# robotseu/ORB_Line_SLAM

Hardware: AMD Instinct MI355X
Metric: stereo frames/s extract+match (ORB+LBD), KITTI 1242x375 (higher is better)
Workload: dtype u8

## Files before the change

### include/orbline.h

```cpp
#ifndef ORBLINE_H
#define ORBLINE_H

#include "orbline_types.h"

#ifdef __cplusplus
extern "C" {
#endif

typedef struct olf_ctx olf_ctx;

const char* olf_last_error(void);
int olf_device_count(void);
int olf_default_params(olf_params* p);

int  olf_ctx_create(const olf_params* p, int width, int height, int max_images, olf_ctx** out);
void olf_ctx_destroy(olf_ctx* ctx);
int  olf_ctx_synchronize(olf_ctx* ctx);
int  olf_ctx_set_input_event(olf_ctx* ctx, void* hip_event);
int  olf_ctx_set_deferred_join(olf_ctx* ctx, int on);
int  olf_stereo_frames_join_dev(olf_ctx* ctx, void* stream);
int  olf_ctx_poll_status(olf_ctx* ctx);

int olf_profile_enable(olf_ctx* ctx, int on);
int olf_profile_reset(olf_ctx* ctx);
// ... 9 lines not shown
                                       float* d_map1, float* d_map2, void* stream);
int olf_init_undistort_rectify_map(olf_ctx* ctx, const double* K, const double* D, int n_dist, const double* R, const double* P, int w, int h,
                                   float* map1, float* map2);
int olf_cvt_gray(olf_ctx* ctx, const uint8_t* src, int code, int n_images, uint8_t* gray);
int olf_remap_linear(olf_ctx* ctx, const uint8_t* src, int src_w, int src_h, const float* mapx, const float* mapy, int dst_w, int dst_h,
                     int n_images, uint8_t* dst);

int olf_distinctive_descriptors(olf_ctx* ctx, const uint8_t* desc, const int32_t* offs, int n_points, int32_t* best);

size_t olf_kf_record_bytes(int n_keys, int n_lines);
int olf_kf_record_pack(uint64_t frame_id, uint64_t kf_id, double timestamp, const float* t3, const float* quat4, int n_keys,
                       const olf_keypoint* keys, const float* uright, const float* depth, const uint8_t* desc, const uint64_t* mappoint_ids,
                       int n_lines, const olf_keyline* lines, const float* disparity2, const double* le3, const uint8_t* ldesc,
                       const uint64_t* mapline_ids, uint8_t* out, size_t capacity, size_t* written);
int olf_kf_record_counts(const uint8_t* buf, size_t len, int32_t* n_keys, int32_t* n_lines, size_t* record_bytes);
int olf_kf_record_unpack(const uint8_t* buf, size_t len, uint64_t* frame_id, uint64_t* kf_id, double* timestamp, float* t3, float* quat4,
                         olf_keypoint* keys, float* uright, float* depth, uint8_t* desc, uint64_t* mappoint_ids, olf_keyline* lines,
                         float* disparity2, double* le3, uint8_t* ldesc, uint64_t* mapline_ids);

typedef struct olf_voc olf_voc;
int olf_voc_create(int k, int L, int scoring, int weighting, int n_nodes, const int32_t* parent, const uint8_t* is_leaf, const uint8_t* desc,
                   const double* weight, olf_voc** out);
int olf_voc_load_text(const char* path, olf_voc** out);
void olf_voc_destroy(olf_voc* voc);
int olf_voc_info(const olf_voc* voc, int* k, int* L, int* scoring, int* weighting, int* n_nodes, int* n_words);
int olf_bow_words_dev(olf_ctx* ctx, const olf_voc* voc, const uint8_t* d_desc, int n, int levelsup, int32_t* d_word, double* d_weight,
                      int32_t* d_node, void* stream);
int olf_bow_assemble(const olf_voc* voc, const int32_t* word, const double* weight, const int32_t* node, int n, int32_t* bow_ids,
                     double* bow_vals, int* n_bow, int32_t* fv_nodes, int32_t* fv_offs, int32_t* fv_idx, int* n_fv);
int olf_bow_transform(olf_ctx* ctx, const olf_voc* voc, const uint8_t* desc, int n, int levelsup, int32_t* bow_ids, double* bow_vals,
                      int* n_bow, int32_t* fv_nodes, int32_t* fv_offs, int32_t* fv_idx, int* n_fv);
int olf_search_by_bow_batch_dev(olf_ctx* ctx, const olf_voc* voc, int n_frames, int img_stride, const olf_keypoint* d_kps, const uint8_t* d_desc,
                                const int32_t* d_counts, const uint8_t* d_mp_valid, const uint8_t* d_mp_bad, float nnratio, int check_orientation,
                                int levelsup, int32_t* d_matches, int32_t* d_nmatches, void* stream);

int olf_orb_scale_tables(const olf_ctx* ctx, float* scale, float* inv_scale, float* sigma2, float* inv_sigma2,
                         int32_t* features_per_level);
int olf_orb_level_sizes(const olf_ctx* ctx, int32_t* widths, int32_t* heights);
int olf_orb_capacity(const olf_ctx* ctx);
int olf_orb_extract_strided(olf_ctx* ctx, const uint8_t* image, size_t row_stride, olf_keypoint* kps, uint8_t* desc, int32_t* count);
int olf_orb_extract_dev(olf_ctx* ctx, const uint8_t* d_images, int n_images, olf_keypoint* d_kps, uint8_t* d_desc,
                        int32_t* d_counts, void* stream);
int olf_orb_extract(olf_ctx* ctx, const uint8_t* images, int n_images, olf_keypoint* kps, uint8_t* desc, int32_t* counts);
int olf_orb_pyramid_level(olf_ctx* ctx, int image, int level, int blurred, uint8_t* dst);
int olf_orb_debug_candidates(olf_ctx* ctx, int image, int level, int32_t* xys, int cap, int32_t* count);
int olf_debug_status(olf_ctx* ctx, int32_t* out64);
int olf_debug_status_n(olf_ctx* ctx, int32_t* out, int n);
int olf_debug_lsd_owner(olf_ctx* ctx, int image, uint32_t* out);
int olf_debug_lsd_regions(olf_ctx* ctx, int image, int32_t* start_n, double* angle, int cap, int32_t* count);
int olf_debug_lsd_waves(olf_ctx* ctx, int waves_per_image, int rob_entries);
int olf_debug_lsd_groups(olf_ctx* ctx, int groups);
int olf_debug_lsd_scatter(olf_ctx* ctx, int on);
int olf_debug_lsd_log_cap(olf_ctx* ctx, int entries);
int olf_debug_seed_sort(olf_ctx* ctx, const uint32_t* keys, int n, int kthr, int depth_limit, uint32_t* out, int32_t* out_n);
int olf_debug_seed_sort_mode(olf_ctx* ctx, int mode);
int olf_debug_seed_sort_wide(olf_ctx* ctx, const uint64_t* keys, int n, int64_t kthr, int depth_limit, int full, uint32_t* out, int32_t* out_n);
int olf_debug_lsd_pool(olf_ctx* ctx, int pool_chunks);
int olf_debug_fdiv_sweep(olf_ctx* ctx, uint64_t seed, int blocks, int per_thread, uint64_t* mismatches);
int olf_debug_sqrtq_sweep(olf_ctx* ctx, int count, uint64_t* mismatches);
int olf_debug_align_sweep(olf_ctx* ctx, uint64_t seed, int blocks, int per_thread, uint64_t* out3);

int olf_stereo_points_dev(olf_ctx* ctx, int n_pairs, const olf_keypoint* d_kps, const uint8_t* d_desc, const int32_t* d_counts,
                          float* d_uright, float* d_depth, void* stream);
int olf_stereo_points(olf_ctx* ctx, const uint8_t* images, int n_pairs, olf_keypoint* kps, uint8_t* desc, int32_t* counts,
                      float* uright, float* depth);

int olf_match_bf_dev(olf_ctx* ctx, const uint8_t* d_descA, const int32_t* d_nA, int strideA, int a_step, const uint8_t* d_descB,
                     const int32_t* d_nB, int strideB, int b_step, int n_sets, float nnr, int best_lr, int32_t* d_m12, void* stream);
int olf_match_bf(olf_ctx* ctx, const uint8_t* descA, int nA, const uint8_t* descB, int nB, float nnr, int best_lr, int32_t* m12);
int olf_knn2(olf_ctx* ctx, const uint8_t* descQ, int nQ, const uint8_t* descT, int nT, int32_t* idx0, int32_t* dist0, int32_t* dist1);
int olf_match_candidates_dev(olf_ctx* ctx, const uint8_t* d_descQ, int nQ, const uint8_t* d_descT, int nT, const int32_t* d_cand_offsets,
                             const int32_t* d_cand_idx, uint16_t* d_dist, void* stream);
int olf_match_candidates(olf_ctx* ctx, const uint8_t* descQ, int nQ, const uint8_t* descT, int nT, const int32_t* cand_offsets,
                         const int32_t* cand_idx, uint16_t* dist);
typedef struct olf_frame_view {
    const olf_keypoint* keys;
    const uint8_t* desc;
    const float*   uright;
    int32_t        n;
    uint8_t*       mp_valid;
    uint8_t*       mp_obs;
    const uint8_t* mp_bad;
    const float*   mp_world;
    const uint8_t* mp_desc;
    const uint8_t* outlier;
    const float*   Tcw;
    float fx, fy, cx, cy, mbf, minX, maxX, minY, maxY;
    const float*   scale_factors;
    int32_t        n_levels;
    const float*   mp_maxd;
    const float*   mp_mind;
    const int32_t* fv_nodes;
    const int32_t* fv_offsets;
    const int32_t* fv_features;
    int32_t        fv_n;
} olf_frame_view;
int olf_search_by_projection(olf_ctx* ctx, const olf_frame_view* cur, const olf_frame_view* last, float th, int bMono, int check_orientation,
                             int32_t* matches, int32_t* nmatches);
int olf_search_by_projection_match12(olf_ctx* ctx, const olf_frame_view* cur, const olf_frame_view* last, float th, int bMono, int check_orientation,
                                     int32_t* matches, int32_t* match12, int32_t* nmatches);
int olf_search_for_initialization(olf_ctx* ctx, const olf_frame_view* f1, const olf_frame_view* f2, float* prev_matched, int window_size,
                                  float nnratio, int check_orientation, int32_t* matches12, int32_t* nmatches);
int olf_search_by_bow(olf_ctx* ctx, const olf_frame_view* kf, const olf_frame_view* f, float nnratio, int check_orientation, int32_t* matched,
                      int32_t* nmatches);
int olf_search_local_map(olf_ctx* ctx, const olf_frame_view* f, int n_mp, const uint8_t* track_in_view, const uint8_t* bad,
                         const int32_t* track_scale_level, const float* track_view_cos, const float* track_proj3, const uint8_t* mp_desc,
// ... 66 lines not shown
```

### orb_line_slam_amd/csrc/api.cpp

```cpp
#include "olf_internal.hpp"
#include "line_internal.hpp"
#include "../../include/orbline.h"
#include <map>
#include <mutex>
#include <cstring>
#include <mutex>

namespace olf {
static thread_local std::string g_err;
void set_error(const std::string& s) { g_err = s; }
}

using namespace olf;

struct olf_ctx {
    olf_params params;
    int W = 0, H = 0, max_images = 0;
    int device = 0;
    hipStream_t stream = nullptr;
    OrbHostTables orb;
    OrbDeviceBufs ob;
    uint8_t* d_images = nullptr;
    olf_keypoint* d_kps = nullptr;
    uint8_t* d_desc = nullptr;
// ... 527 lines not shown
    if (hipMalloc(&b, bytes) != hipSuccess) { (void)hipFree(a); set_error("olf_debug_copy_bandwidth: hipMalloc failed"); return OLF_ERR_HIP; }
    hipEvent_t e0, e1;
    (void)hipEventCreate(&e0); (void)hipEventCreate(&e1);
    (void)hipMemsetAsync(a, 1, bytes, c->stream);
    int rc = olf::launch_copy16(a, b, bytes, c->stream);
    (void)hipEventRecord(e0, c->stream);
    for (int i = 0; i < reps && rc == OLF_OK; ++i) rc = olf::launch_copy16(i & 1 ? b : a, i & 1 ? a : b, bytes, c->stream);
    (void)hipEventRecord(e1, c->stream);
    const hipError_t se = hipEventSynchronize(e1);
    float ms = 0.f;
    (void)hipEventElapsedTime(&ms, e0, e1);
    (void)hipEventDestroy(e0); (void)hipEventDestroy(e1); (void)hipFree(a); (void)hipFree(b);
    if (rc != OLF_OK || se != hipSuccess || !(ms > 0)) { set_error("olf_debug_copy_bandwidth: copy failed"); return OLF_ERR_HIP; }
    *gbytes_per_s = 2.0 * (double)(bytes / 16 * 16) * reps / (ms * 1e-3) / 1e9;
    return OLF_OK;
}

int olf_debug_lsd_waves(olf_ctx* c, int waves_per_image, int rob_entries)
{
    const bool pow2 = rob_entries > 0 && (rob_entries & (rob_entries - 1)) == 0;
    if (!c || waves_per_image > 16 || waves_per_image < -1 || (rob_entries != 0 && (!pow2 || rob_entries < 128 || rob_entries > 1024))) {
        set_error("olf_debug_lsd_waves: bad argument"); return OLF_ERR_INVALID;
    }
    c->lsd_force.waves = waves_per_image;
    c->lsd_force.robEntries = rob_entries;
    return OLF_OK;
}

int olf_debug_lsd_groups(olf_ctx* c, int groups)
{
    if (!c || !(groups == 0 || groups == 1 || groups == 2 || groups == 4)) { set_error("olf_debug_lsd_groups: bad argument"); return OLF_ERR_INVALID; }
    c->lsd_force.groups = groups > 0 ? groups : -1;
    return OLF_OK;
}

int olf_debug_lsd_log_cap(olf_ctx* c, int entries)
{
    if (!c || entries < 0) { set_error("olf_debug_lsd_log_cap: bad argument"); return OLF_ERR_INVALID; }
    OLF_TRY(check_device(c, "olf_debug_lsd_log_cap"));
    LineGeom& g = c->line.geom;
    if (entries > 0 && !g.spillArena) {
        const size_t blocks = std::max<size_t>(2, (size_t)c->max_images - (size_t)c->max_images / 4);
        void* q = nullptr;
        OLF_HIP_CHECK(hipMalloc(&q, blocks * 8 * (size_t)g.Ps));
        c->allocs.push_back(q);
        g.spillArena = static_cast<uint32_t*>(q); g.spillBlocks = (int)blocks;
    }
    g.logCap = entries > 0 ? std::min(entries, g.regionStride / 2) : g.regionStride / 2;
    OLF_HIP_CHECK(hipDeviceSynchronize());
    OLF_HIP_CHECK(hipMemcpy(c->lb.geom, &g, sizeof(LineGeom), hipMemcpyHostToDevice));
    return OLF_OK;
}

int olf_debug_lsd_scatter(olf_ctx* c, int on)
{
    if (!c) { set_error("olf_debug_lsd_scatter: bad argument"); return OLF_ERR_INVALID; }
    c->lsd_force.scatter = on ? 1 : 0;
    return OLF_OK;
}

int olf_debug_seed_sort(olf_ctx* c, const uint32_t* keys, int n, int kthr, int depth_limit, uint32_t* out, int32_t* out_n)
{
    if (!c || !keys || !out || !out_n || n < 0 || n > c->line.geom.Ps || kthr < 0 || kthr > 1023) { set_error("olf_debug_seed_sort: bad argument"); return OLF_ERR_INVALID; }
    OLF_HIP_CHECK(hipMemcpyAsync(c->lb.keysA, keys, (size_t)n * 4, hipMemcpyHostToDevice, c->stream));
    OLF_TRY(launch_lsd_seedsort(c->line.geom, c->lb, lsd_plan(c->line.geom, c->lb, c->lsd_force, c->limits, 1), 1, c->stream, n, kthr, depth_limit));
    int cnt = 0;
    OLF_HIP_CHECK(hipMemcpyAsync(&cnt, c->lb.keyCount, sizeof(int), hipMemcpyDeviceToHost, c->stream));
    OLF_HIP_CHECK(hipStreamSynchronize(c->stream));
    *out_n = cnt;
    if (cnt < 0 || cnt > n) { set_error("olf_debug_seed_sort: count out of range"); return OLF_ERR_HIP; }
    if (cnt) OLF_HIP_CHECK(hipMemcpy(out, c->lb.keysB, (size_t)cnt * 4, hipMemcpyDeviceToHost));
    return OLF_OK;
}

int olf_debug_seed_sort_wide(olf_ctx* c, const uint64_t* keys, int n, int64_t kthr, int depth_limit, int full, uint32_t* out, int32_t* out_n)
{
    if (!c || !keys || !out || !out_n || n < 0 || n > c->line.geom.Ps || kthr < 0 || kthr > 0xffffffffll || !c->line.geom.wide) {
        set_error("olf_debug_seed_sort_wide: bad argument (the context must be a wide one: lsd_n_bins > 1024 or 2^22 pixels and more)"); return OLF_ERR_INVALID; }
    OLF_HIP_CHECK(hipMemcpyAsync(c->lb.keysA, keys, (size_t)n * 8, hipMemcpyHostToDevice, c->stream));
    OLF_TRY(launch_lsd_sort_wide(c->line.geom, c->lb, 1, c->stream, n, (long long)kthr, depth_limit, full ? 1 : 0));
    int cnt = 0;
    OLF_HIP_CHECK(hipMemcpyAsync(&cnt, c->lb.keyCount, sizeof(int), hipMemcpyDeviceToHost, c->stream));
    OLF_HIP_CHECK(hipStreamSynchronize(c->stream));
    *out_n = cnt;
    if (cnt < 0 || cnt > n) { set_error("olf_debug_seed_sort_wide: count out of range"); return OLF_ERR_HIP; }
    if (cnt) OLF_HIP_CHECK(hipMemcpy(out, c->lb.keysB, (size_t)cnt * 4, hipMemcpyDeviceToHost));
    return check_status(c);
}

int olf_debug_seed_sort_mode(olf_ctx* c, int mode)
{
    if (!c || mode < -1 || mode == 3 || mode == 4 || mode > 5) { set_error("olf_debug_seed_sort_mode: bad argument"); return OLF_ERR_INVALID; }
    c->lsd_force.sortMode = mode;
    return OLF_OK;
}

int olf_debug_lsd_pool(olf_ctx* c, int pool_chunks)
{
    if (!c || pool_chunks < 0) { set_error("olf_debug_lsd_pool: bad argument"); return OLF_ERR_INVALID; }
    c->lsd_force.poolChunks = pool_chunks;
    return OLF_OK;
}

int olf_debug_lsd_regions(olf_ctx* c, int image, int32_t* start_n , double* angle, int cap, int32_t* count)
{
    if (!c || !start_n || !angle || !count || image < 0 || image >= c->max_images) return OLF_ERR_INVALID;
// ... 544 lines not shown
```

### orb_line_slam_amd/csrc/line_internal.hpp

```cpp
#pragma once
#include "olf_internal.hpp"

namespace olf {

struct LineGeom {
    int W, H, pitchW;
    int Ws, Hs, pitchS, Ps;
    int nThr;
    int nBins;
    int wide;
    int minRegSize;
    double prec;
    double precWrap;
    double scale;
    double minLength;
    int maxDetect;
    int rectGrid;
    int maxRegions;
    int nFeatures;
    int outCap;
    int pitchD;
    int lsdTaps[7];
    int lsdWideR;
    int lsdWide[15];
// ... 11 lines not shown
    float alignTanLo, alignTanHi;
    float alignDeg;
    int regionStride;
    int resizeExact;
    int logCap;
    int spillBlocks;
    uint32_t* spillArena;
    int* spillCtl;
    int* spillOf;
};

struct LineDeviceBufs {
    uint8_t* lsdBlur = nullptr;
    uint8_t* scaled = nullptr;
    uint32_t* grad = nullptr;
    uint32_t* keysA = nullptr;
    uint32_t* keysB = nullptr;
    int* keyCount = nullptr;
    int* maxN = nullptr;
    int* chunkCnt = nullptr;
    uint32_t* region = nullptr;
    olf_keyline* rawLines = nullptr;
    int* rawCount = nullptr;
    int* regCount = nullptr;
    uint8_t* lbdBlur = nullptr;
    uint32_t* dxdy = nullptr;
    float* rowSums = nullptr;
    float* lbdStarts = nullptr;
    ResizeCoef* rx = nullptr;
    ResizeCoef* ry = nullptr;
    LineGeom* geom = nullptr;
    uint32_t* sortHist = nullptr;
    uint32_t* sortBase = nullptr;
    int* status = nullptr;
    float* angDeg = nullptr;
    void* angEnt = nullptr;
    int ownerImages = 0;
    uint32_t* owner = nullptr;
    int* links = nullptr;
    int nChunks = 0;
    int* growFmt = nullptr;
    int* topBuf = nullptr;
    unsigned char* mg = nullptr;
    size_t mgStride = 0;
    int mgImages = 0;
};

struct LsdOverrides {
    int sortMode = -1;
    int waves = -1, robEntries = 0;
    int groups = -1;
    int poolChunks = 0;
    int scatter = 0;
};

struct DeviceLimits { int nCU = 64, maxLds = 64 * 1024; };

struct LsdPlan {
    enum Resize { Upgrad, Tiled, Upsample } resize;
    enum Sort { Radix, Seed, Wide } sort;
    bool keysOwner, keysAll;
    int sortWaves;
    bool sortTop; int sortGroups;
    int growWaves;
    int robEntries, growGroups, poolChunks, scatter;
    int agentRefine, agentPF, agentLaunches;
    enum Rect { Emit, Mixed, Plain } rect;
};
LsdPlan lsd_plan(const LineGeom& g, const LineDeviceBufs& b, const LsdOverrides& o, const DeviceLimits& d, int n_images);

constexpr int kBatchCtxImages = 2048;

struct LineHostTables {
    LineGeom geom;
    std::vector<ResizeCoef> rx, ry;
    int build(const olf_line_params& p, int W, int H, int max_images = 2);
};

int launch_lsd_front(const LineGeom& g, const LineDeviceBufs& b, const LsdPlan& p, const uint8_t* d_in, int in_pitch, int n_images, hipStream_t s,
                     hipEvent_t sortEvent, bool writeScaled);
int launch_lsd_grow(const LineGeom& g, const LineDeviceBufs& b, const LsdPlan& p, int n_images, hipStream_t s);
int launch_lsd_rect(const LineGeom& g, const LineDeviceBufs& b, const LsdPlan& p, int n_images, hipStream_t s);
int launch_lbd_dense(const LineGeom& g, const LineDeviceBufs& b, const uint8_t* d_in, int in_pitch, int n_images, hipStream_t s);
int launch_line_select_lbd(const LineGeom& g, const LineDeviceBufs& b, const uint8_t* d_in, int in_pitch, int n_images,
                           olf_keyline* d_kls, uint8_t* d_desc, int* d_counts, hipStream_t s, bool denseDone = false);
int launch_lbd_only(const LineGeom& g, const LineDeviceBufs& b, const uint8_t* d_in, int in_pitch, int n_images, const olf_keyline* d_kls,
                    uint8_t* d_desc, const int* d_counts, hipStream_t s);
int launch_gauss7_img(const uint8_t* src, int srcPitch, size_t srcStride, uint8_t* dst, int dstPitch, size_t dstStride, int W, int H,
                      const LineGeom& g, int which, int n_images, hipStream_t s);
int launch_lsd_angle_table(LineDeviceBufs& b, int libmFloat, hipStream_t s);
int launch_fdiv_sweep(unsigned long long seed, int blocks, int per_thread, unsigned long long* d_mismatches, hipStream_t s);
int launch_sqrtq_sweep(int count, unsigned long long* d_mismatches, hipStream_t s);
int launch_align_sweep(const LineDeviceBufs& b, unsigned long long seed, int blocks, int per_thread, unsigned long long* d_out, hipStream_t s);
int lsd_sort_max_chunks(int Ps);
size_t lsd_grow_mg_stride(int maxRegions);
constexpr int kMwMaxImages = 3072;
constexpr int kMgMaxImages = 64;
int launch_lsd_grow_mw(const LineGeom& g, const LineDeviceBufs& b, const LsdPlan& p, int n_images, hipStream_t s);
int lsd_seedsort_top_words();
int launch_lsd_sort(const LineGeom& g, const LineDeviceBufs& b, int n_images, hipStream_t s);
int launch_lsd_seedsort(const LineGeom& g, const LineDeviceBufs& b, const LsdPlan& p, int n_images, hipStream_t s, int nOverride, int kthrOverride, int depthOverride);
int launch_lsd_sort_wide(const LineGeom& g, const LineDeviceBufs& b, int n_images, hipStream_t s, int nOverride, long long kthrOverride, int depthOverride, int fullOverride);

size_t stereo_lines_prep_bytes(int n_images, int cap);
int launch_stereo_lines(int W, int H, const olf_stereo_params& P, int n_pairs, const olf_keyline* d_kls, const uint8_t* d_desc,
                        const int* d_counts, int cap, void* d_prep, uint16_t* d_dist , int* d_m21, int* d_m12,
                        float* d_disp, double* d_le, hipStream_t s);

}
```

### orb_line_slam_amd/csrc/lsd.hip

```cpp
#include "lsd_device.hpp"

namespace olf {


__device__ __forceinline__ int refl101(int p, int n)
{
    if (p < 0) p = -p;
    if (p >= n) p = 2 * (n - 1) - p;
    return p;
}

int launch_gauss7_img(const uint8_t* src, int srcPitch, size_t srcStride, uint8_t* dst, int dstPitch, size_t dstStride, int W, int H,
                      const LineGeom& g, int which, int n_images, hipStream_t s)
{
    if (!which && g.lsdWideR > 3) return launch_sep_wide(src, srcStride, srcPitch, dst, dstStride, dstPitch, W, H, g.lsdWide, g.lsdWideR, n_images, s);
    return launch_sep7(src, srcStride, srcPitch, dst, dstStride, dstPitch, W, H, which ? g.lbdTaps : g.lsdTaps, n_images, s);
}

__global__ __launch_bounds__(256) void k_lsd_upsample(const uint8_t* __restrict__ src, uint8_t* __restrict__ dst,
                                                      const LineGeom* __restrict__ gp, const ResizeCoef* __restrict__ rx,
                                                      const ResizeCoef* __restrict__ ry)
{
    const LineGeom& g = *gp;
    const int img = blockIdx.y;
// ... 1274 lines not shown
                        }
                        ++nreg;
                    } else if (lane == 0) atomicOr(status, 8);
                }
            }
            if (!REFINE && n >= minRegSize) {
                if (nreg < maxRegions) {
                    if (lane == 0) {
                        RegionRec rr; rr.start = rbase; rr.n = n; rr.angle = reg_angle;
                        recs[nreg] = rr;
                    }
                    ++nreg;
                    rbase += n;
                } else if (lane == 0) atomicOr(status, 8);
            }
#ifdef OLF_STATS
            st_acc += n; if (n >= minRegSize) st_logged += n; if (n > 1) st_regl += __popcll(wave_vote(valid && lane > l));
#endif
            if (REFINE && maskEpoch != flushEpoch) {
                const uint32_t wnow = valid ? grad[addr] : kUsed;
                mask = wave_vote(valid && lane > l && !(wnow & (kUsed | kNotDef)) && s_pend[addr & (PEND - 1)] != addr);
                if (wave_bit(mask)) wseed = wnow;
                if (wave_bit(mask & ~tabM) && !isoSeed) { const AngEnt* t = ent + (wseed & 0x3fffffu); seedAng = t->ang; seedSum = t->seed; }
                tabM |= mask;
                maskEpoch = flushEpoch;
            }
            else if (n == 1) mask &= mask - 1;
            else if (PIPE || maskEpoch == flushEpoch) {
                mask &= ~((2ull << l) - 1ull) & wave_vote(s_pend[addr & (PEND - 1)] != addr);
            } else {
                mask = wave_vote(valid && lane > l && !(grad[addr] & (kUsed | kNotDef)) && s_pend[addr & (PEND - 1)] != addr);
                maskEpoch = flushEpoch;
            }
        }
        if (PFSEED) asm volatile("" :: "v"(pfA), "v"(pfB));
    }
#undef ALIGN_CHEAP
#undef ENSURE_ANGLE
#undef LOG_ROOM
#undef LOG_AT
#undef MARK_USED
#undef PEND_FLUSH
#undef PEND_CLEAR
#ifdef OLF_STATS
    if (lane == 0 && img == 0) { long long* o = reinterpret_cast<long long*>(status + 16); o[0] = st_rounds; o[1] = st_k; o[2] = st_t; o[3] = st_full; o[4] = st_single; o[5] = st_rounds_big; o[6] = st_k_big; o[7] = st_t_big;
        o[8] = st_flush; o[9] = st_iters; o[10] = st_deep1; o[11] = st_deep2; o[12] = st_cand; o[13] = st_regions; o[14] = st_mem;
        o[15] = nkeys; o[16] = st_win; o[17] = st_seedl; o[18] = st_regl; o[19] = st_acc; o[20] = st_isos; o[21] = st_logged; o[22] = st_winLive; o[23] = st_first; o[24] = st_cand1;
        o[25] = st_acc1; o[26] = st_wentries; o[27] = st_whand; o[28] = st_wdone; o[29] = st_wpend; }
#endif
    if (lane == 0) { regCount[img] = over ? 0 : nreg; if (growFmt) growFmt[img] = 1; if (g.spillOf && !retry) g.spillOf[img] = over ? -1 : 0; }
}


template <bool CHAINED>
__device__ __forceinline__ void lsd_rect_region(const LineGeom& g, int img, int r, const uint32_t* __restrict__ gradAll,
                                                const uint32_t* __restrict__ regionAll, const RegionRec* __restrict__ recsAll,
                                                SegCand* __restrict__ candAll, const int* __restrict__ linksAll, int nChunks, const int* __restrict__ spillOf,
                                                const uint32_t* __restrict__ spillArena)
{
    const uint32_t* grad = gradAll + (size_t)img * g.Ps;
    const RegionRec rr = recsAll[(size_t)img * g.maxRegions + r];
    const uint32_t* px_list = CHAINED ? regionAll + (size_t)img * nChunks * 32 : nullptr;
    const int sblk = CHAINED || !spillOf ? 0 : spillOf[img];
    const uint2* log2 = CHAINED ? nullptr
                      : (sblk > 0 ? reinterpret_cast<const uint2*>(spillArena) + (size_t)(sblk - 1) * g.Ps
                                  : reinterpret_cast<const uint2*>(regionAll + (size_t)img * g.regionStride)) + rr.start;
    const int* links = CHAINED ? linksAll + (size_t)img * nChunks : nullptr;
    const int n = rr.n, Ws = g.Ws;
    int cid = rr.start, nxt = -1;
#define RECT_BLOCK(q0) (px_list + (size_t)cid * 32 + ((q0) & 31))
#define RECT_STEP(q0) do { if (CHAINED) { if (((q0) & 31) == 0) { if (q0) cid = nxt; nxt = links[cid]; } } } while (0)
    constexpr int U = 16;
    double x = 0, y = 0, sum = 0;
    for (int q0 = 0; q0 < n; q0 += U) {
        uint32_t rp[U], p[U];
        if (CHAINED) {
            RECT_STEP(q0);
            const uint32_t* blk = RECT_BLOCK(q0);
#pragma unroll
            for (int u = 0; u < U; ++u) rp[u] = q0 + u < n ? blk[u] : 0u;
#pragma unroll
            for (int u = 0; u < U; ++u) p[u] = grad[(int)(rp[u] >> 16) * Ws + (int)(rp[u] & 0xffffu)];
        } else {
#pragma unroll
            for (int u = 0; u < U; u += 2) {
                uint4 e = make_uint4(0u, 0u, 0u, 0u);
                if (q0 + u + 1 < n) __builtin_memcpy(&e, log2 + q0 + u, 16);
                else if (q0 + u < n) { const uint2 e1 = log2[q0 + u]; e.x = e1.x; e.y = e1.y; }
                rp[u] = e.x; p[u] = e.y; rp[u + 1] = e.z; p[u + 1] = e.w;
            }
        }
#pragma unroll
        for (int u = 0; u < U; ++u) {
            if (q0 + u < n) {
                const int px = (int)(rp[u] & 0xffffu), py = (int)(rp[u] >> 16);
                const int gx = unpack_gx(p[u]), gy = unpack_gy(p[u]);
                const double wt = sqrt_quarter(gx * gx + gy * gy);
                x = d_add(x, d_mul((double)px, wt));
                y = d_add(y, d_mul((double)py, wt));
                sum = d_add(sum, wt);
            }
        }
    }
    x = x / sum; y = y / sum;
    double Ixx = 0, Iyy = 0, Ixy = 0;
    cid = rr.start;
    for (int q0 = 0; q0 < n; q0 += U) {
        uint32_t rp[U], p[U];
        if (CHAINED) {
            RECT_STEP(q0);
            const uint32_t* blk = RECT_BLOCK(q0);
#pragma unroll
            for (int u = 0; u < U; ++u) rp[u] = q0 + u < n ? blk[u] : 0u;
#pragma unroll
            for (int u = 0; u < U; ++u) p[u] = grad[(int)(rp[u] >> 16) * Ws + (int)(rp[u] & 0xffffu)];
        } else {
#pragma unroll
            for (int u = 0; u < U; u += 2) {
                uint4 e = make_uint4(0u, 0u, 0u, 0u);
                if (q0 + u + 1 < n) __builtin_memcpy(&e, log2 + q0 + u, 16);
                else if (q0 + u < n) { const uint2 e1 = log2[q0 + u]; e.x = e1.x; e.y = e1.y; }
                rp[u] = e.x; p[u] = e.y; rp[u + 1] = e.z; p[u + 1] = e.w;
            }
        }
#pragma unroll
        for (int u = 0; u < U; ++u) {
            if (q0 + u < n) {
                const int px = (int)(rp[u] & 0xffffu), py = (int)(rp[u] >> 16);
                const int gx = unpack_gx(p[u]), gy = unpack_gy(p[u]);
                const double wt = sqrt_quarter(gx * gx + gy * gy);
                const double ex = d_sub((double)px, x), ey = d_sub((double)py, y);
                Ixx = d_add(Ixx, d_mul(d_mul(ey, ey), wt));
                Iyy = d_add(Iyy, d_mul(d_mul(ex, ex), wt));
                Ixy = d_sub(Ixy, d_mul(d_mul(ex, ey), wt));
            }
        }
    }
    const double dI = d_sub(Ixx, Iyy);
    const double lambda = d_mul(0.5, d_sub(d_add(Ixx, Iyy), sqrt(d_add(d_mul(dI, dI), d_mul(d_mul(4.0, Ixy), Ixy)))));
    double theta = (fabs(Ixx) > fabs(Iyy)) ? (double)dev_fastAtan2((float)d_sub(lambda, Ixx), (float)Ixy)
                                           : (double)dev_fastAtan2((float)Ixy, (float)d_sub(lambda, Iyy));
    theta = d_mul(theta, kDegToRads);
    {
        double diff = d_sub(theta, rr.angle);
        while (diff <= -kPI) diff = d_add(diff, kM2PI);
        while (diff > kPI) diff = d_sub(diff, kM2PI);
        if (fabs(diff) > g.prec) theta = d_add(theta, kPI);
    }
    double ddx, ddy;
    sincos(theta, &ddy, &ddx);
    double l_min = 0, l_max = 0;
    cid = rr.start;
    for (int q0 = 0; q0 < n; q0 += U) {
        uint32_t rp[U];
        if (CHAINED) {
            RECT_STEP(q0);
            const uint32_t* blk = RECT_BLOCK(q0);
#pragma unroll
            for (int u = 0; u < U; ++u) rp[u] = q0 + u < n ? blk[u] : 0u;
        } else {
#pragma unroll
            for (int u = 0; u < U; u += 2) {
                uint4 e = make_uint4(0u, 0u, 0u, 0u);
                if (q0 + u + 1 < n) __builtin_memcpy(&e, log2 + q0 + u, 16);
                else if (q0 + u < n) e.x = log2[q0 + u].x;
                rp[u] = e.x; rp[u + 1] = e.z;
            }
        }
#pragma unroll
        for (int u = 0; u < U; ++u) {
            if (q0 + u < n) {
                const double rdx = d_sub((double)(int)(rp[u] & 0xffffu), x), rdy = d_sub((double)(int)(rp[u] >> 16), y);
                const double lq = d_add(d_mul(rdx, ddx), d_mul(rdy, ddy));
                l_max = fmax(l_max, lq); l_min = fmin(l_min, lq);
            }
        }
    }
    double x1 = d_add(x, d_mul(l_min, ddx)), y1 = d_add(y, d_mul(l_min, ddy));
    double x2 = d_add(x, d_mul(l_max, ddx)), y2 = d_add(y, d_mul(l_max, ddy));
    const SegCand c = rect_to_cand(g, x1, y1, x2, y2);
    candAll[(size_t)img * g.maxRegions + r] = c;
#undef RECT_BLOCK
#undef RECT_STEP
}

template <bool CHAINED>
__global__ __launch_bounds__(256) void k_lsd_rect(const LineGeom* __restrict__ gp, const uint32_t* __restrict__ gradAll,
                                                  const uint32_t* __restrict__ regionAll, const RegionRec* __restrict__ recsAll,
                                                  const int* __restrict__ regCount, SegCand* __restrict__ candAll,
                                                  const int* __restrict__ linksAll, int nChunks, const int* __restrict__ spillOf, const uint32_t* __restrict__ spillArena)
{
    const int img = blockIdx.y, r = blockIdx.x * 256 + threadIdx.x;
    if (r >= regCount[img]) return;
    lsd_rect_region<CHAINED>(*gp, img, r, gradAll, regionAll, recsAll, candAll, linksAll, nChunks, spillOf, spillArena);
}

__global__ __launch_bounds__(256) void k_lsd_rect_mixed(const LineGeom* __restrict__ gp, const uint32_t* __restrict__ gradAll,
                                                        const uint32_t* __restrict__ regionAll, const RegionRec* __restrict__ recsAll,
                                                        const int* __restrict__ regCount, SegCand* __restrict__ candAll,
                                                        const int* __restrict__ linksAll, int nChunks, const int* __restrict__ growFmt, const int* __restrict__ spillOf,
                                                        const uint32_t* __restrict__ spillArena)
{
    const int img = blockIdx.y, r = blockIdx.x * 256 + threadIdx.x;
    if (r >= regCount[img]) return;
    if (growFmt[img] == 1) lsd_rect_region<false>(*gp, img, r, gradAll, regionAll, recsAll, candAll, linksAll, nChunks, spillOf, spillArena);
    else lsd_rect_region<true>(*gp, img, r, gradAll, regionAll, recsAll, candAll, linksAll, nChunks, spillOf, spillArena);
}

__global__ __launch_bounds__(256) void k_lsd_emit(const LineGeom* __restrict__ gp, const SegCand* __restrict__ candAll, const int* __restrict__ regCount,
                                                  olf_keyline* __restrict__ rawLines, int* __restrict__ rawCount, int* __restrict__ status)
{
    __shared__ int s_wave[4];
    __shared__ int s_base;
    const LineGeom& g = *gp;
    const int img = blockIdx.x, tid = threadIdx.x, lane = tid & 63, wave = tid >> 6;
    const SegCand* cand = candAll + (size_t)img * g.maxRegions;
    olf_keyline* out = rawLines + (size_t)img * g.maxDetect;
    const int nreg = regCount[img];
    if (tid == 0) s_base = 0;
    __syncthreads();
    for (int r0 = 0; r0 < nreg; r0 += 256) {
        const int r = r0 + tid;
        SegCand c; c.keep = 0;
        if (r < nreg) c = cand[r];
        const unsigned long long km = wave_vote(c.keep != 0);
        if (lane == 0) s_wave[wave] = __popcll(km);
        __syncthreads();
        int pos = s_base + wave_rank_below(km);
        for (int w = 0; w < wave; ++w) pos += s_wave[w];
        if (c.keep) {
            if (pos < g.maxDetect) {
                const float e0 = c.e0, e1 = c.e1, e2 = c.e2, e3 = c.e3;
                olf_keyline kl;
                kl.startPointX = e0; kl.startPointY = e1; kl.endPointX = e2; kl.endPointY = e3;
                kl.sPointInOctaveX = e0; kl.sPointInOctaveY = e1; kl.ePointInOctaveX = e2; kl.ePointInOctaveY = e3;
                kl.lineLength = c.length;
                const int rx1 = __float2int_rn(e0), ry1 = __float2int_rn(e1), rx2 = __float2int_rn(e2), ry2 = __float2int_rn(e3);
                kl.numOfPixels = max(abs(rx2 - rx1), abs(ry2 - ry1)) + 1;
                kl.angle = g.libmFloat ? glibc_atan2f(f_sub(e3, e1), f_sub(e2, e0)) : (float)atan2((double)f_sub(e3, e1), (double)f_sub(e2, e0));
                kl.class_id = pos; kl.octave = 0;
                kl.size = f_mul(f_sub(e2, e0), f_sub(e3, e1));
                kl.response = f_div(kl.lineLength, (float)max(g.W, g.H));
                kl.pt_x = f_div(f_add(e2, e0), 2.0f); kl.pt_y = f_div(f_add(e3, e1), 2.0f);
                out[pos] = kl;
            } else atomicOr(status, 8);
        }
        __syncthreads();
        if (tid == 0) s_base += s_wave[0] + s_wave[1] + s_wave[2] + s_wave[3];
        __syncthreads();
    }
    if (tid == 0) rawCount[img] = min(s_base, g.maxDetect);
}

LsdPlan lsd_plan(const LineGeom& g, const LineDeviceBufs& b, const LsdOverrides& o, const DeviceLimits& d, int n)
{
    LsdPlan p{};
    p.resize = (g.resizeTiled & 4) && g.seedOrder == 1 ? LsdPlan::Upgrad : g.resizeTiled ? LsdPlan::Tiled : LsdPlan::Upsample;
    p.sort = g.wide ? LsdPlan::Wide : g.seedOrder == 1 ? LsdPlan::Seed : LsdPlan::Radix;
    p.keysAll = g.seedOrder == 1;

    const int m = o.sortMode;
    p.sortWaves = m < 0 ? (n <= 256 ? 8 : n <= 640 ? 4 : n <= 1536 ? 2 : 1) : m == 2 ? 8 : m == 1 ? 4 : m == 5 ? 2 : 1;
    auto sortLds = [](int w) { return w == 8 ? 104 * 1024 : w == 4 ? 56 * 1024 : w == 2 ? 32 * 1024 : 0; };
    while (sortLds(p.sortWaves) > d.maxLds) p.sortWaves /= 2;
    p.sortTop = p.sortWaves > 1 && b.topBuf && n <= 64;
    p.sortGroups = !p.sortTop ? 1 : n <= 16 ? 8 : 4;

    const int autoWaves = n <= 512 ? 16 : n <= 1024 ? 8
                        : n <= 1536 ? 4
                        : n <= 2048 ? 8 : n <= kMwMaxImages ? 4
                        : 0;
    p.growWaves = (g.refine || g.wide || n > b.ownerImages) ? 0 : o.waves >= 0 ? o.waves : autoWaves;
    p.keysOwner = p.growWaves > 0;
    if (p.growWaves > 0) {
        const int nw = p.growWaves;
        p.robEntries = o.robEntries > 0 ? o.robEntries : (nw >= 16 ? 512 : nw >= 8 ? 256 : 128);
        p.poolChunks = o.poolChunks > 0 ? std::min(o.poolChunks, b.nChunks) : b.nChunks;
        int G = o.groups > 0 ? o.groups : nw >= 16 && n <= kMgMaxImages ? 2 : 1;
        while (G > 1 && (!b.mg || n > b.mgImages || n * G > d.nCU || p.poolChunks / G < p.robEntries + 64)) G >>= 1;
        p.growGroups = G;
        p.scatter = o.scatter;
        p.agentRefine = 0; p.agentPF = 0; p.agentLaunches = 1;
    } else {
        p.agentRefine = g.refine;
        p.agentPF = (g.wide ? 32 : 0) | (g.refine ? 0 : g.alignTanLo < 0.f ? 11 : 27);
        p.agentLaunches = g.logCap < g.Ps ? 2 : 1;
    }
    p.rect = g.refine ? LsdPlan::Emit : p.growWaves > 0 ? LsdPlan::Mixed : LsdPlan::Plain;
    return p;
}

int launch_lsd_front(const LineGeom& g, const LineDeviceBufs& b, const LsdPlan& p, const uint8_t* d_in, int in_pitch, int n_images, hipStream_t s,
                     hipEvent_t sortEvent, bool writeScaled)
{
    OLF_HIP_CHECK(hipMemsetAsync(b.maxN, 0, (size_t)n_images * 32 * sizeof(int), s));
    OLF_HIP_CHECK(hipMemsetAsync(b.keyCount, 0, (size_t)n_images * 32 * sizeof(int), s));
    { int rc = launch_gauss7_img(d_in, in_pitch, (size_t)in_pitch * g.H, b.lsdBlur, g.pitchW, (size_t)g.pitchW * g.H, g.W, g.H, g, 0, n_images, s);
      if (rc != OLF_OK) return rc; }
    if (p.resize == LsdPlan::Upgrad) {
        const int nsx = (g.Ws + 3) / 4;
        hipLaunchKernelGGL(k_lsd_upgrad, dim3((nsx + 63) / 64, (g.Hs + UG_ROWS - 1) / UG_ROWS, n_images), dim3(64), 0, s, b.lsdBlur, b.scaled, b.grad, b.geom, b.rx, b.ry,
                           b.maxN, nsx, writeScaled ? 1 : 0);
    } else if (p.resize == LsdPlan::Tiled) {
        int rc = launch_resize_tiled(b.lsdBlur, (size_t)g.pitchW * g.H, g.pitchW, g.W, g.H, b.scaled, (size_t)g.pitchS * g.Hs, g.pitchS, g.Ws, g.Hs, b.rx,
                                     b.ry, n_images, s, (g.resizeTiled & 2) != 0);
        if (rc != OLF_OK) return rc;
    } else {
        const int quads = ((g.Ws + 3) >> 2) * g.Hs;
        hipLaunchKernelGGL(k_lsd_upsample, dim3((quads + 255) / 256, n_images), dim3(256), 0, s, b.lsdBlur, b.scaled, b.geom, b.rx, b.ry);
    }
    if (p.resize != LsdPlan::Upgrad) hipLaunchKernelGGL(k_lsd_grad, dim3((g.Ps + LG_CHUNK - 1) / LG_CHUNK, n_images), dim3(256), 0, s, b.scaled, b.grad, b.geom, b.maxN, b.chunkCnt);
    {
        const int nChunks = (g.Ps + LG_CHUNK - 1) / LG_CHUNK, total = nChunks * n_images;
        const size_t lds = (size_t)(LG_CHUNK + 2 * g.Ws + 2) * sizeof(float);
        if (lds > 60 * 1024) { set_error("LSD image wider than the key kernel's LDS window"); return OLF_ERR_CAPACITY; }
        const auto keys = p.sort == LsdPlan::Wide ? (p.keysAll ? k_lsd_keys<false, true, LG_CHUNK, true> : k_lsd_keys<false, false, LG_CHUNK, true>)
                        : p.keysAll ? (p.keysOwner ? k_lsd_keys<true, true, LG_CHUNK> : k_lsd_keys<false, true, LG_CHUNK>)
                        : p.keysOwner ? k_lsd_keys<true, false, LG_CHUNK> : k_lsd_keys<false, false, LG_CHUNK>;
        hipLaunchKernelGGL(keys, dim3(total), dim3(KEYS_THREADS), lds, s, b.grad, b.geom, b.maxN, b.chunkCnt, p.sort == LsdPlan::Radix ? b.keysB : b.keysA, b.keyCount,
                           b.owner, b.angDeg, nChunks, total);
    }
    OLF_HIP_CHECK(hipGetLastError());
    if (sortEvent) OLF_HIP_CHECK(hipEventRecord(sortEvent, s));
    if (p.sort == LsdPlan::Wide) return launch_lsd_sort_wide(g, b, n_images, s, -1, -1, -1, -1);
    if (p.sort == LsdPlan::Seed) return launch_lsd_seedsort(g, b, p, n_images, s, -1, -1, -1);
    return launch_lsd_sort(g, b, n_images, s);
}

int launch_lsd_grow(const LineGeom& g, const LineDeviceBufs& b, const LsdPlan& p, int n_images, hipStream_t s)
{
    static const struct { int refine, pf; decltype(&k_lsd_grow<0, 0>) kernel; } kAgents[] = {
        {0, 0, k_lsd_grow<0, 0>}, {2, 32, k_lsd_grow<2, 32>}, {1, 32, k_lsd_grow<1, 32>}, {0, 32 | 11, k_lsd_grow<0, 32 | 11>}, {0, 32 | 27, k_lsd_grow<0, 32 | 27>},
        {2, 0, k_lsd_grow<2, 0>}, {1, 0, k_lsd_grow<1, 0>}, {0, 11, k_lsd_grow<0, 11>}, {0, 27, k_lsd_grow<0, 27>}};
    decltype(&k_lsd_grow<0, 0>) agent = nullptr;
    for (const auto& a : kAgents) if (a.refine == p.agentRefine && a.pf == p.agentPF) agent = a.kernel;
    if (!agent) { set_error("launch_lsd_grow: no such k_lsd_grow instantiation"); return OLF_ERR_INVALID; }
    if (g.spillCtl) OLF_HIP_CHECK(hipMemsetAsync(g.spillCtl, 0, sizeof(int), s));
    if (p.growWaves > 0) { const int rc = launch_lsd_grow_mw(g, b, p, n_images, s); if (rc != OLF_OK) return rc; }
    for (int retry = 0; retry < p.agentLaunches; ++retry)
        hipLaunchKernelGGL(agent, dim3(n_images), dim3(64), 0, s, b.geom, b.grad, b.keysB, b.keyCount, b.region,
                           p.agentRefine ? (RegionRec*)nullptr : reinterpret_cast<RegionRec*>(b.keysA), b.regCount, b.status, reinterpret_cast<const AngEnt*>(b.angEnt),
                           p.growWaves > 0 ? b.growFmt : (int*)nullptr, p.agentRefine ? reinterpret_cast<SegCand*>(b.keysA) : (SegCand*)nullptr, retry);
    OLF_HIP_CHECK(hipGetLastError());
    return OLF_OK;
}

int launch_lsd_rect(const LineGeom& g, const LineDeviceBufs& b, const LsdPlan& p, int n_images, hipStream_t s)
{
    if (p.rect == LsdPlan::Emit) {
        hipLaunchKernelGGL(k_lsd_emit, dim3(n_images), dim3(256), 0, s, b.geom, reinterpret_cast<const SegCand*>(b.keysA), b.regCount, b.rawLines,
                           b.rawCount, b.status);
        OLF_HIP_CHECK(hipGetLastError());
        return OLF_OK;
    }
    const int* spillOf = g.logCap < g.Ps ? g.spillOf : nullptr;
    if (p.rect == LsdPlan::Mixed)
        hipLaunchKernelGGL(k_lsd_rect_mixed, dim3((g.rectGrid + 255) / 256, n_images), dim3(256), 0, s, b.geom, b.grad, b.region,
                           reinterpret_cast<const RegionRec*>(b.keysA), b.regCount, reinterpret_cast<SegCand*>(b.keysB), b.links, b.nChunks, b.growFmt, spillOf, g.spillArena);
    else
        hipLaunchKernelGGL(k_lsd_rect<false>, dim3((g.rectGrid + 255) / 256, n_images), dim3(256), 0, s, b.geom, b.grad, b.region,
                           reinterpret_cast<const RegionRec*>(b.keysA), b.regCount, reinterpret_cast<SegCand*>(b.keysB), b.links, b.nChunks, spillOf, g.spillArena);
    hipLaunchKernelGGL(k_lsd_emit, dim3(n_images), dim3(256), 0, s, b.geom, reinterpret_cast<const SegCand*>(b.keysB), b.regCount, b.rawLines,
                       b.rawCount, b.status);
    OLF_HIP_CHECK(hipGetLastError());
    return OLF_OK;
}

}
```

Before: 15160.

## Add wave-cooperative LDS-staged rectangle kernel for plain LSD rect path

```diff
diff --git a/include/orbline.h b/include/orbline.h
--- a/include/orbline.h
+++ b/include/orbline.h
@@ -85,6 +85,7 @@
 int olf_debug_lsd_groups(olf_ctx* ctx, int groups);
 int olf_debug_lsd_scatter(olf_ctx* ctx, int on);
 int olf_debug_lsd_log_cap(olf_ctx* ctx, int entries);
+int olf_debug_lsd_rect_cap(olf_ctx* ctx, int entries);
 int olf_debug_seed_sort(olf_ctx* ctx, const uint32_t* keys, int n, int kthr, int depth_limit, uint32_t* out, int32_t* out_n);
 int olf_debug_seed_sort_mode(olf_ctx* ctx, int mode);
 int olf_debug_seed_sort_wide(olf_ctx* ctx, const uint64_t* keys, int n, int64_t kthr, int depth_limit, int full, uint32_t* out, int32_t* out_n);
diff --git a/orb_line_slam_amd/csrc/api.cpp b/orb_line_slam_amd/csrc/api.cpp
--- a/orb_line_slam_amd/csrc/api.cpp
+++ b/orb_line_slam_amd/csrc/api.cpp
@@ -603,6 +603,13 @@
     return OLF_OK;
 }
 
+int olf_debug_lsd_rect_cap(olf_ctx* c, int entries)
+{
+    if (!c || entries < 0 || entries > lsd_rect_slice()) { set_error("olf_debug_lsd_rect_cap: bad argument"); return OLF_ERR_INVALID; }
+    c->lsd_force.rectCap = entries;
+    return OLF_OK;
+}
+
 int olf_debug_lsd_scatter(olf_ctx* c, int on)
 {
     if (!c) { set_error("olf_debug_lsd_scatter: bad argument"); return OLF_ERR_INVALID; }
diff --git a/orb_line_slam_amd/csrc/line_internal.hpp b/orb_line_slam_amd/csrc/line_internal.hpp
--- a/orb_line_slam_amd/csrc/line_internal.hpp
+++ b/orb_line_slam_amd/csrc/line_internal.hpp
@@ -87,6 +87,7 @@
     int groups = -1;
     int poolChunks = 0;
     int scatter = 0;
+    int rectCap = 0;
 };
 
 struct DeviceLimits { int nCU = 64, maxLds = 64 * 1024; };
@@ -101,6 +102,7 @@
     int robEntries, growGroups, poolChunks, scatter;
     int agentRefine, agentPF, agentLaunches;
     enum Rect { Emit, Mixed, Plain } rect;
+    int rectCap;
 };
 LsdPlan lsd_plan(const LineGeom& g, const LineDeviceBufs& b, const LsdOverrides& o, const DeviceLimits& d, int n_images);
 
@@ -116,6 +118,7 @@
                      hipEvent_t sortEvent, bool writeScaled);
 int launch_lsd_grow(const LineGeom& g, const LineDeviceBufs& b, const LsdPlan& p, int n_images, hipStream_t s);
 int launch_lsd_rect(const LineGeom& g, const LineDeviceBufs& b, const LsdPlan& p, int n_images, hipStream_t s);
+int lsd_rect_slice();
 int launch_lbd_dense(const LineGeom& g, const LineDeviceBufs& b, const uint8_t* d_in, int in_pitch, int n_images, hipStream_t s);
 int launch_line_select_lbd(const LineGeom& g, const LineDeviceBufs& b, const uint8_t* d_in, int in_pitch, int n_images,
                            olf_keyline* d_kls, uint8_t* d_desc, int* d_counts, hipStream_t s, bool denseDone = false);
diff --git a/orb_line_slam_amd/csrc/lsd.hip b/orb_line_slam_amd/csrc/lsd.hip
--- a/orb_line_slam_amd/csrc/lsd.hip
+++ b/orb_line_slam_amd/csrc/lsd.hip
@@ -1350,6 +1350,20 @@
 }
 
 
+__device__ __forceinline__ double rect_theta(double Ixx, double Iyy, double Ixy, double reg_angle, double prec)
+{
+    const double dI = d_sub(Ixx, Iyy);
+    const double lambda = d_mul(0.5, d_sub(d_add(Ixx, Iyy), sqrt(d_add(d_mul(dI, dI), d_mul(d_mul(4.0, Ixy), Ixy)))));
+    double theta = (fabs(Ixx) > fabs(Iyy)) ? (double)dev_fastAtan2((float)d_sub(lambda, Ixx), (float)Ixy)
+                                           : (double)dev_fastAtan2((float)Ixy, (float)d_sub(lambda, Iyy));
+    theta = d_mul(theta, kDegToRads);
+    double diff = d_sub(theta, reg_angle);
+    while (diff <= -kPI) diff = d_add(diff, kM2PI);
+    while (diff > kPI) diff = d_sub(diff, kM2PI);
+    if (fabs(diff) > prec) theta = d_add(theta, kPI);
+    return theta;
+}
+
 template <bool CHAINED>
 __device__ __forceinline__ void lsd_rect_region(const LineGeom& g, int img, int r, const uint32_t* __restrict__ gradAll,
                                                 const uint32_t* __restrict__ regionAll, const RegionRec* __restrict__ recsAll,
@@ -1434,17 +1448,7 @@
             }
         }
     }
-    const double dI = d_sub(Ixx, Iyy);
-    const double lambda = d_mul(0.5, d_sub(d_add(Ixx, Iyy), sqrt(d_add(d_mul(dI, dI), d_mul(d_mul(4.0, Ixy), Ixy)))));
-    double theta = (fabs(Ixx) > fabs(Iyy)) ? (double)dev_fastAtan2((float)d_sub(lambda, Ixx), (float)Ixy)
-                                           : (double)dev_fastAtan2((float)Ixy, (float)d_sub(lambda, Iyy));
-    theta = d_mul(theta, kDegToRads);
-    {
-        double diff = d_sub(theta, rr.angle);
-        while (diff <= -kPI) diff = d_add(diff, kM2PI);
-        while (diff > kPI) diff = d_sub(diff, kM2PI);
-        if (fabs(diff) > g.prec) theta = d_add(theta, kPI);
-    }
+    const double theta = rect_theta(Ixx, Iyy, Ixy, rr.angle, g.prec);
     double ddx, ddy;
     sincos(theta, &ddy, &ddx);
     double l_min = 0, l_max = 0;
@@ -1491,6 +1495,130 @@
     const int img = blockIdx.y, r = blockIdx.x * 256 + threadIdx.x;
     if (r >= regCount[img]) return;
     lsd_rect_region<CHAINED>(*gp, img, r, gradAll, regionAll, recsAll, candAll, linksAll, nChunks, spillOf, spillArena);
+}
+
+#ifndef OLF_RECT_SLICE
+#define OLF_RECT_SLICE 2048
+#endif
+constexpr int kRectSlice = OLF_RECT_SLICE;
+int lsd_rect_slice() { return kRectSlice; }
+
+__global__ __launch_bounds__(64) void k_lsd_rect_span(const LineGeom* __restrict__ gp, const uint32_t* __restrict__ regionAll,
+                                                      const RegionRec* __restrict__ recsAll, const int* __restrict__ regCount, SegCand* __restrict__ candAll,
+                                                      const int* __restrict__ spillOf, const uint32_t* __restrict__ spillArena, int cap)
+{
+    __shared__ uint4 s_pair[kRectSlice / 2];
+    const uint2* s_ent = reinterpret_cast<const uint2*>(s_pair);
+    const LineGeom& g = *gp;
+    const int img = blockIdx.y, r0 = blockIdx.x * 64, lane = threadIdx.x;
+    const int nreg = regCount[img];
+    if (r0 >= nreg) return;
+    const int r = r0 + lane;
+    const bool live = r < nreg;
+    RegionRec rr; rr.start = 0; rr.n = 0; rr.angle = 0;
+    if (live) rr = recsAll[(size_t)img * g.maxRegions + r];
+    const int sblk = spillOf ? spillOf[img] : 0;
+    const uint2* log2 = sblk > 0 ? reinterpret_cast<const uint2*>(spillArena) + (size_t)(sblk - 1) * g.Ps
+                                 : reinterpret_cast<const uint2*>(regionAll + (size_t)img * g.regionStride);
+    const int start = rr.start, end = rr.start + rr.n;
+    int span0 = __builtin_amdgcn_readfirstlane(start);
+    const int spanEnd = -wave_min_i32(-end);
+    if (span0 > 0 && ((reinterpret_cast<uintptr_t>(log2 + span0) >> 3) & 1)) --span0;
+    int have = -1;
+#define RECT_STAGE(c0, c1) do { \
+        if (have != (c0)) { \
+            __syncthreads(); \
+            for (int eb = (c0); eb < (c1); eb += 8 * 128) { \
+                uint4 v[8]; \
+                _Pragma("unroll") for (int i = 0; i < 8; ++i) { \
+                    const int e = eb + i * 128 + 2 * lane; \
+                    v[i] = make_uint4(0u, 0u, 0u, 0u); \
+                    if (e + 1 < (c1)) __builtin_memcpy(&v[i], log2 + e, 16); \
+                    else if (e < (c1)) { const uint2 e1 = log2[e]; v[i].x = e1.x; v[i].y = e1.y; } \
+                } \
+                _Pragma("unroll") for (int i = 0; i < 8; ++i) { \
+                    const int e = eb + i * 128 + 2 * lane; \
+                    if (e < (c1)) s_pair[(e - (c0)) >> 1] = v[i]; \
+                } \
+            } \
+            __syncthreads(); \
+            have = (c0); \
+        } } while (0)
+    constexpr int U = 8;
+    double x = 0, y = 0, sum = 0;
+    for (int c0 = span0; c0 < spanEnd; c0 += cap) {
+        const int c1 = min(c0 + cap, spanEnd);
+        RECT_STAGE(c0, c1);
+        const int qhi = min(end, c1) - c0;
+        for (int q0 = max(start, c0) - c0; q0 < qhi; q0 += U) {
+            uint2 e[U];
+#pragma unroll
+            for (int u = 0; u < U; ++u) e[u] = s_ent[min(q0 + u, qhi - 1)];
+#pragma unroll
+            for (int u = 0; u < U; ++u) {
+                if (q0 + u < qhi) {
+                    const int px = (int)(e[u].x & 0xffffu), py = (int)(e[u].x >> 16);
+                    const int gx = unpack_gx(e[u].y), gy = unpack_gy(e[u].y);
+                    const double wt = sqrt_quarter(gx * gx + gy * gy);
+                    x = d_add(x, d_mul((double)px, wt));
+                    y = d_add(y, d_mul((double)py, wt));
+                    sum = d_add(sum, wt);
+                }
+            }
+        }
+    }
+    if (!live) sum = 1.0;
+    x = x / sum; y = y / sum;
+    double Ixx = 0, Iyy = 0, Ixy = 0;
+    for (int c0 = span0; c0 < spanEnd; c0 += cap) {
+        const int c1 = min(c0 + cap, spanEnd);
+        RECT_STAGE(c0, c1);
+        const int qhi = min(end, c1) - c0;
+        for (int q0 = max(start, c0) - c0; q0 < qhi; q0 += U) {
+            uint2 e[U];
+#pragma unroll
+            for (int u = 0; u < U; ++u) e[u] = s_ent[min(q0 + u, qhi - 1)];
+#pragma unroll
+            for (int u = 0; u < U; ++u) {
+                if (q0 + u < qhi) {
+                    const int px = (int)(e[u].x & 0xffffu), py = (int)(e[u].x >> 16);
+                    const int gx = unpack_gx(e[u].y), gy = unpack_gy(e[u].y);
+                    const double wt = sqrt_quarter(gx * gx + gy * gy);
+                    const double ex = d_sub((double)px, x), ey = d_sub((double)py, y);
+                    Ixx = d_add(Ixx, d_mul(d_mul(ey, ey), wt));
+                    Iyy = d_add(Iyy, d_mul(d_mul(ex, ex), wt));
+                    Ixy = d_sub(Ixy, d_mul(d_mul(ex, ey), wt));
+                }
+            }
+        }
+    }
+    const double theta = rect_theta(Ixx, Iyy, Ixy, rr.angle, g.prec);
+    double ddx, ddy;
+    sincos(theta, &ddy, &ddx);
+    double l_min = 0, l_max = 0;
+    for (int c0 = span0; c0 < spanEnd; c0 += cap) {
+        const int c1 = min(c0 + cap, spanEnd);
+        RECT_STAGE(c0, c1);
+        const int qhi = min(end, c1) - c0;
+        for (int q0 = max(start, c0) - c0; q0 < qhi; q0 += U) {
+            uint32_t rp[U];
+#pragma unroll
+            for (int u = 0; u < U; ++u) rp[u] = s_ent[min(q0 + u, qhi - 1)].x;
+#pragma unroll
+            for (int u = 0; u < U; ++u) {
+                if (q0 + u < qhi) {
+                    const double rdx = d_sub((double)(int)(rp[u] & 0xffffu), x), rdy = d_sub((double)(int)(rp[u] >> 16), y);
+                    const double lq = d_add(d_mul(rdx, ddx), d_mul(rdy, ddy));
+                    l_max = fmax(l_max, lq); l_min = fmin(l_min, lq);
+                }
+            }
+        }
+    }
+#undef RECT_STAGE
+    if (!live) return;
+    double x1 = d_add(x, d_mul(l_min, ddx)), y1 = d_add(y, d_mul(l_min, ddy));
+    double x2 = d_add(x, d_mul(l_max, ddx)), y2 = d_add(y, d_mul(l_max, ddy));
+    candAll[(size_t)img * g.maxRegions + r] = rect_to_cand(g, x1, y1, x2, y2);
 }
 
 __global__ __launch_bounds__(256) void k_lsd_rect_mixed(const LineGeom* __restrict__ gp, const uint32_t* __restrict__ gradAll,
@@ -1585,6 +1713,7 @@
         p.agentLaunches = g.logCap < g.Ps ? 2 : 1;
     }
     p.rect = g.refine ? LsdPlan::Emit : p.growWaves > 0 ? LsdPlan::Mixed : LsdPlan::Plain;
+    p.rectCap = p.rect != LsdPlan::Plain || kRectSlice * 8 > d.maxLds ? 0 : o.rectCap > 0 ? std::min(o.rectCap, kRectSlice) : kRectSlice;
     return p;
 }
 
@@ -1655,6 +1784,9 @@
     if (p.rect == LsdPlan::Mixed)
         hipLaunchKernelGGL(k_lsd_rect_mixed, dim3((g.rectGrid + 255) / 256, n_images), dim3(256), 0, s, b.geom, b.grad, b.region,
                            reinterpret_cast<const RegionRec*>(b.keysA), b.regCount, reinterpret_cast<SegCand*>(b.keysB), b.links, b.nChunks, b.growFmt, spillOf, g.spillArena);
+    else if (p.rectCap > 0)
+        hipLaunchKernelGGL(k_lsd_rect_span, dim3((g.rectGrid + 63) / 64, n_images), dim3(64), 0, s, b.geom, b.region, reinterpret_cast<const RegionRec*>(b.keysA),
+                           b.regCount, reinterpret_cast<SegCand*>(b.keysB), spillOf, g.spillArena, p.rectCap);
     else
         hipLaunchKernelGGL(k_lsd_rect<false>, dim3((g.rectGrid + 255) / 256, n_images), dim3(256), 0, s, b.geom, b.grad, b.region,
                            reinterpret_cast<const RegionRec*>(b.keysA), b.regCount, reinterpret_cast<SegCand*>(b.keysB), b.links, b.nChunks, spillOf, g.spillArena);
```

Result: slower. 14330 (-5.5%).
